# francescovidaich964/TensorNetworkForML

Measured on AMD Instinct MI355X. Metric: sweep-steps/sec, 28x28 MNIST-shaped, bond=20, batch=5000 per GPU, higher is better.
Workload: dtype f32; 1 GPU; c3: N=784 sites, D=2, L=2, bond 20, batch 5000/GPU, softmax+full_cross_ent, trunc=fixed, L2_flag=True; pass = hand-over of one of 4 staged batches + forward + 783-step sweep; global_batch=5000, sweep_steps_per_pass=783, parallelism=dp1, distinct_batches=4

## Files before the change

### tensornetworkforml_amd/csrc/kernels_narrow.hip

```cpp
#include "tnml_internal.h"
#include "jacobi_device.h"
#include "small_gemm_device.h"
#include "wide_pipe_device.h"

namespace tnml {

__device__ inline double wave_sum_f64(double v) {
  v += dpp_f64<0xB1>(v);
  v += dpp_f64<0x4E>(v);
  v += dpp_f64<0x141>(v);
  v += dpp_f64<0x140>(v);
  const double r0 = wave_read_f64(v, 0), r1 = wave_read_f64(v, 16), r2 = wave_read_f64(v, 32), r3 = wave_read_f64(v, 48);
  return (r0 + r1) + (r2 + r3);
}

template <int BUF>
__device__ inline void block_sum3(double &a, double &b, double &c, double *scratch) {
  const int lane = threadIdx.x & 63, wave = threadIdx.x >> 6, nw = blockDim.x >> 6;
  double *s = scratch + BUF * 64;
  a = wave_sum_f64(a); b = wave_sum_f64(b); c = wave_sum_f64(c);
  if (lane == 0) { s[wave] = a; s[16 + wave] = b; s[32 + wave] = c; }
  lds_barrier();
  const int w = lane & 15;
  double ta = w < nw ? s[w] : 0.0, tb = w < nw ? s[16 + w] : 0.0, tc = w < nw ? s[32 + w] : 0.0;
// ... 792 lines not shown
        if (round_idx - __builtin_amdgcn_readfirstlane(last_big1) >= ne - 1) { converged = 1; break; }
      }
      if (!converged) kept2 = kept_scale(Gc);
    }
  } else {
    converged = 1;
  }
  double *V = V0;
  if (vLaneOk) {
#pragma unroll
    for (int r = 0; r < kVR; ++r) {
      const int P = vP0 + r;
      if (r < vr && P < np) {
        *reinterpret_cast<double2 *>(V + (2 * P) * ne + 2 * vQ) = make_double2(vb[r][0], vb[r][1]);
        *reinterpret_cast<double2 *>(V + (2 * P + 1) * ne + 2 * vQ) = make_double2(vb[r][2], vb[r][3]);
      }
    }
  }
  if (p.stamps && tid == 0) t_c2 = __builtin_amdgcn_s_memtime();

  for (int j = tid; j < n; j += NT) k.dLam[j] = __builtin_amdgcn_ldexp(fmax(Gc[j * ne + j], 0.0), sc_exp);
  lds_barrier();
  if (use_chol) {
    for (int j = tid; j < n; j += NT) {
      const double ls = Gc[j * ne + j];
      k.dSq[j] = ls > 1e-300 ? 1.0 / sqrt(ls) : 0.0;
    }
    lds_barrier();
    mm_lds(1, n, n, n, Lm, 0, 1, ne, V, 0, ne, 1, [&](int, int i, int j, double v) { Gn[i * ne + j] = v * k.dSq[j]; });
    V = Gn;
    lds_barrier();
  }
  for (int j = wave_u; j < n; j += NT >> 6) {
    const int i = tid & 63;
    const double lj = k.dLam[j];
    const double li = i < n ? k.dLam[i] : 0.0;
    const int rank = __popcll(__ballot(i < n && ((li > lj) || (li == lj && i < j))));
    if (i == 0) {
      k.sOrd[rank] = j;
      if (p.dbg) p.dbg[4 * (size_t)Bs + rank] = sqrt(lj);
    }
  }
  if (tid == 0) {
    if (p.counters) {
      atomicAdd(p.counters, (unsigned long long)sweeps);
      atomicAdd(p.counters + 1, 1ull);
      atomicAdd(p.counters + 2, (unsigned long long)round_idx);
      if (use_chol) atomicAdd(p.counters + 3, 1ull);
    }
    if (!converged) atomicOr(p.status, 2);
    if (p.dbg) {
      double *sc = p.dbg + 4 * (size_t)Bs + kDbgSigma;
      sc[3] = (double)sweeps;
      sc[4] = (double)n;
    }
  }
  lds_barrier();

  if (p.stamps && tid == 0) t_c2b = __builtin_amdgcn_s_memtime();
  int mk = m, ob_s_h = p.ob_s_h, ob_s_d = p.ob_s_d, oa_s_d = p.oa_s_d, oa_s_g = p.oa_s_g;
  const int ob_s_m = p.ob_s_m, oa_s_m = p.oa_s_m;
  float *const out_behind = p.out_behind, *const out_ahead = p.out_ahead;
  double *const Nh_new = p.Nh_new;
  if (p.trunc_thr > 0.0) {
    if (tid == 0) {
      double tot = 0.0;
      for (int j = 0; j < n; ++j) tot += sqrt(k.dLam[k.sOrd[j]]);
      double cum = 0.0;
      int idx = 0;
      bool found = false;
      for (int j = 0; j < n && !found; ++j) {
        cum += sqrt(k.dLam[k.sOrd[j]]);
// ... 13 lines not shown
    const double lam = k.dLam[k.sOrd[sp]];
    const bool ok = lam > 1e-300 && lam > 1e-30 * lam_max;
    const double sq = ok ? sqrt(sqrt(lam)) : 0.0;
    k.dSq[sp] = sq;
    k.dSq[ne + sp] = ok ? 1.0 / sq : 0.0;
  }
  lds_barrier();
  for (int kk = wave_u; kk < n; kk += NT >> 6)
   for (int sp = tid & 63; sp < mk; sp += 64) {
    const int j = k.sOrd[sp];
    const double vq = V[kk * ne + j];
    const float v = (float)(vq * k.dSq[sp]);
    k.dVs[kk * mk + sp] = vq * k.dSq[ne + sp];
    if (short_rows) {
      k.sCb[kk * mk + sp] = v;
      if (p.persist) PL.Ad[kk * mk + sp] = vq * k.dSq[sp];
      st_behind((kk / D) * ob_s_h + (kk % D) * ob_s_d + sp * ob_s_m, v);
    } else {
      const int l = kk % L, q = kk / L;
      out_ahead[sp * oa_s_m + (q / g) * oa_s_d + (q % g) * oa_s_g + l] = v;
    }
   }
  lds_barrier();
  const int DM = D * mk;
  auto store_T2 = [&](int, int i, int j, double v) { k.dT2[i * DM + j] = v; };
  if (short_rows) {
    int slot = 0;
    if (!p.persist || p.write_ahead)
      slot = mm_lds(L, D * g, mk, n, k.fB, 1, L, c, k.dVs, 0, mk, 1,
           [&](int l, int qq, int sp, double acc) {
             const int dk1 = qq >= g ? 1 : 0;
             out_ahead[__mul24(sp, oa_s_m) + dk1 * oa_s_d + __mul24(qq - dk1 * g, oa_s_g) + l] = (float)acc;
           });
    if (Nh_new) mm_lds(1, h, DM, h, k.dNh, 0, h, 1, k.sCb, 0, DM, 1, store_T2, false, slot);
  } else {
    mm_lds(D, h, mk, n, k.fBp, c + 1, D * (c + 1), 1, k.dVs, 0, mk, 1,
           [&](int dk, int h_, int sp, double acc) {
             const float v = (float)acc;
             k.sCb[__mul24(h_ * D + dk, mk) + sp] = v;
             if (p.persist) PL.Ad[__mul24(h_ * D + dk, mk) + sp] = acc;
             st_behind(__mul24(h_, ob_s_h) + dk * ob_s_d + __mul24(sp, ob_s_m), v);
           });
  }
  lds_barrier();
  if (p.persist) {
    if (wave_u == (NT >> 6) - 1) {
      const int ln = tid & 63;
      const __amdgpu_buffer_rsrc_t rP = sc1_rsrc(p.Apub);
      for (int e = ln; e < (r * mk) >> 1; e += 64) st_sc1_b128(rP, (unsigned)e * 16u, pack_d2(PL.Ad[2 * e], PL.Ad[2 * e + 1]));
      for (int e = ln; e < (mk + 1) >> 1; e += 64) {
        const double i0 = k.dSq[ne + 2 * e], i1 = 2 * e + 1 < mk ? k.dSq[ne + 2 * e + 1] : 0.0;
        st_sc1_b128(rP, (unsigned)(r * mk + 2 * e) * 8u, pack_d2(i0 * i0, i1 * i1));
      }
      asm volatile("s_waitcnt vmcnt(0)" ::: "memory");
      if (ln == 0) { unsigned *const aflag = p.aflag; __hip_atomic_store(aflag, (unsigned)p.coretoken, __ATOMIC_RELAXED, __HIP_MEMORY_SCOPE_AGENT); }
    }
  }

  if (p.stamps && tid == 0) t_c2c = __builtin_amdgcn_s_memtime();
  if (Nh_new) {
    if (!short_rows) {
      mm_lds(1, h, DM, h, k.dNh, 0, h, 1, k.sCb, 0, DM, 1, store_T2);
      lds_barrier();
    }
    mm_lds(1, mk, mk, h * D, k.sCb, 0, 1, mk, k.dT2, 0, mk, 1,
           [&](int, int i, int j, double v) {
             Nh_new[i * mk + j] = v;
             if (p.persist) PL.Nh[i * mk + j] = v;
           });
    if (p.persist) {
      lds_barrier();
      const __amdgpu_buffer_rsrc_t rP = sc1_rsrc(p.Apub);
      const int oN = persist_pub_off(r * mk, mk), nn2 = mk * mk;
      for (int e = tid; e < (nn2 + 1) >> 1; e += NT)
        st_sc1_b128(rP, (unsigned)(oN + 2 * e) * 8u, pack_d2(PL.Nh[2 * e], 2 * e + 1 < nn2 ? PL.Nh[2 * e + 1] : 0.0));
    }
  }

  if (p.stamps && tid == 0) {
    const unsigned long long t_c3 = __builtin_amdgcn_s_memtime(), t_r3 = __builtin_amdgcn_s_memrealtime();
    p.stamps[0] = (double)(t_c1 - t_c0); p.stamps[1] = (double)(t_c2 - t_c1); p.stamps[2] = (double)(t_c3 - t_c2);
    p.stamps[3] = (double)(t_r3 - t_r0); p.stamps[4] = (double)sweeps; p.stamps[5] = (double)n;
    p.stamps[50] = (double)round_idx;
    for (int i = 0; i < 5; ++i) p.stamps[9 + i] = (double)(t_p[i] - (i ? t_p[i - 1] : t_c0));
    p.stamps[6] = (double)(t_c2b - t_c2); p.stamps[7] = (double)(t_c2c - t_c2b); p.stamps[8] = (double)(t_c3 - t_c2c);
  }

  if (tid == 0 && p.metrics) {
    const double cnt = (double)ldtail(3);
    const double inv = cnt > 0 ? 1.0 / cnt : 0.0;
    p.metrics[0] = (float)((double)ldtail(0) * inv);
// ... 117 lines not shown
      const int nT = nr * DG * L;
      double *Tdst = t.T + (size_t)r0 * DG * L, *Ndst = t.TN + (size_t)r0 * DG * L;
      for (int e = tid; e < nT; e += NT) __hip_atomic_store(Tdst + e, oT[e], __ATOMIC_RELAXED, __HIP_MEMORY_SCOPE_AGENT);
      if (t.l2_flag) {
        lds_barrier();
        for (int e = tid; e < nT; e += NT) __hip_atomic_store(Ndst + e, oN[e], __ATOMIC_RELAXED, __HIP_MEMORY_SCOPE_AGENT);
      }
    }
    asm volatile("s_waitcnt vmcnt(0)" ::: "memory");
    lds_barrier();
    if (tid == 0) __hip_atomic_fetch_add(t.tcnt, 1u, __ATOMIC_RELAXED, __HIP_MEMORY_SCOPE_AGENT);
    return false;
  }
  const int cw = (RW + nH - 1) / nH, c0 = min(RW, hid * cw), nc = min(RW, c0 + cw) - c0;
  const int cw2 = 2 * cw;
  double *sA = (double *)smem_raw;
  double *sIv = sA + (((size_t)zr * h + 1) & ~(size_t)1);
  double *sNh = sIv + ((h + 1) & ~1);
  double *sS = sNh + (((size_t)h * h + 1) & ~(size_t)1);
  float *sOut = (float *)(sS + persist_helper_ss_doubles(zr, h, cw));
  double *sP2 = (double *)sOut + (size_t)h * cw;
  float *sZf = (float *)(sP2 + (size_t)h * cw);
  float *sAff = sZf + (size_t)zr * cw;
  double *hst = (t.stamps && hid == 0 && tid == 0) ? t.stamps : nullptr;
  double *hst2 = (t.stamps && hid == 0) ? t.stamps : nullptr;
  auto rt = []() { return (double)(__builtin_amdgcn_s_memrealtime() & ((1ull << 40) - 1)); };
  if (tid == 0) { if (hst) hst[22] = rt(); give_up(spin_wait_ge(t.tcnt, (unsigned)nH, t.abort_flag)); if (hst) hst[30] = rt(); }
  lds_barrier();
  if (sBad) return true;
  for (int e = tid; e < zr * nc; e += NT) {
    const int i = e / nc, cc = e - i * nc;
    const size_t src = (size_t)i * RW + c0 + cc;
    sS[i * cw2 + cc] = __hip_atomic_load(t.T + src, __ATOMIC_RELAXED, __HIP_MEMORY_SCOPE_AGENT);
    sS[i * cw2 + cw + cc] = t.l2_flag ? __hip_atomic_load(t.TN + src, __ATOMIC_RELAXED, __HIP_MEMORY_SCOPE_AGENT) : 0.0;
  }
  lds_barrier();
  if (tid == 0) { give_up(spin_wait_ge(t.zready, t.zwant, t.abort_flag)); if (hst) hst[24] = rt(); }
  lds_barrier();
  if (sBad) return true;
  for (int e = tid; e < zr * nc; e += NT) {
    const int i = e / nc, cc = e - i * nc;
    sZf[i * cw + cc] = ld_sc1(t.Z + (size_t)i * RW + c0 + cc);
  }
  lds_barrier();
  if (tid == 0) { give_up(t.awant ? spin_wait_ge(t.aflag, t.awant, t.abort_flag) : 0); if (hst) hst[23] = rt(); }
  lds_barrier();
  if (sBad) return true;
  if (t.awant) {
    const __amdgpu_buffer_rsrc_t rP = sc1_rsrc(t.Apub);
    const int n1 = persist_pub_off(zr * h, h) >> 1, nA = (zr * h) >> 1;
    for (int e = tid; e < n1; e += NT) {
      const tn_uvec4 q = ld_sc1_b128(rP, (unsigned)e * 16u);
      *reinterpret_cast<tn_uvec4 *>(sA + 2 * e) = q;
      if (e < nA) { const dvec2_t a = __builtin_bit_cast(dvec2_t, q); sAff[2 * e] = (float)a[0]; sAff[2 * e + 1] = (float)a[1]; }
    }
  } else if (tid == 0) {
    sA[0] = 1.0; sAff[0] = 1.f; sIv[0] = 1.0; sNh[0] = 1.0;
  }
  lds_barrier();
  if (hst) hst[25] = rt();
  if (nc > 0) {
    mm_lds_f32(h, nc, zr, sAff, 1, h, sZf, cw, 1, [&](int i, int j, float v) { sOut[i * cw + j] = v; });
    const int slot = (((h + 15) >> 4) * ((nc + 15) >> 4)) & ((NT >> 6) - 1);
    mm_lds(1, h, t.l2_flag ? 2 * cw : cw, zr, sA, 0, 1, h, sS, 0, cw2, 1,
           [&](int, int i, int j, double v) {
             if (j < cw) { if (j < nc) sOut[(h + i) * cw + j] = (float)(v * sIv[i]); }
             else sP2[i * cw + (j - cw)] = v * sIv[i];
           }, false, slot);
  }
  if (t.l2_flag) {
    if (t.awant && (tid >> 6) == (NT >> 6) - 1) {
      const int ln = tid & 63;
      int bad = 0;
      if (ln == 0) { if (hst2) hst2[31] = rt(); bad = spin_wait_ge(t.nflag, t.awant, t.abort_flag); give_up(bad); if (hst2) hst2[21] = rt(); }
      if (!__builtin_amdgcn_readfirstlane(bad)) {
        const __amdgpu_buffer_rsrc_t rP = sc1_rsrc(t.Apub);
        const int oN = persist_pub_off(zr * h, h), nq = (h * h + 1) >> 1;
        for (int e0 = ln; e0 < nq; e0 += 4 * 64) {
          tn_uvec4 q[4];
#pragma unroll
          for (int u = 0; u < 4; ++u) if (e0 + 64 * u < nq) q[u] = ld_sc1_b128(rP, (unsigned)(oN + 2 * (e0 + 64 * u)) * 8u);
#pragma unroll
          for (int u = 0; u < 4; ++u) if (e0 + 64 * u < nq) *reinterpret_cast<tn_uvec4 *>(sNh + 2 * (e0 + 64 * u)) = q[u];
        }
      }
    }
  }
  lds_barrier();
  if (t.l2_flag && sBad) return true;
  st_sc1_rows(t.prepRaw, sOut, h, cw, RW, c0, nc);
  st_sc1_rows(t.prepB, sOut + (size_t)h * cw, h, cw, RW, c0, nc);
  if (t.l2_flag) {
    if (nc > 0) {
      mm_lds(1, h, nc, h, sNh, 0, 1, h, sP2, 0, cw, 1, [&](int, int i, int j, double v) { sS[i * cw + j] = v; });
    }
    lds_barrier();
    st_sc1_rows(t.prepG, sS, h, cw, RW, c0, nc);
  }
  if (hst) hst[26] = rt();
  asm volatile("s_waitcnt vmcnt(0)" ::: "memory");
  lds_barrier();
  if (tid == 0) __hip_atomic_fetch_add(t.pcnt, 1u, __ATOMIC_RELAXED, __HIP_MEMORY_SCOPE_AGENT);
  if (hst) hst[27] = rt();
  return false;
}

__global__ __launch_bounds__(kNarrowThreads) void sweep_persist_kernel(const PersistStep *__restrict__ steps_g, int n_steps, int nH) {
// ... 109 lines not shown
```

### tensornetworkforml_amd/csrc/san/hip_stub.cpp

```cpp
#include <hip/hip_runtime.h>
#include <rccl/rccl.h>
#include <sys/mman.h>
#include <cstdarg>
#include <cstdio>
#include <cstdlib>
#include <cstring>
#include <map>
#include <string>
#include <vector>
#include <cxxabi.h>
#include "../tnml_internal.h"
#include "../wide_pipe_device.h"

using namespace tnml;

namespace san {
static char *g_base = nullptr;
static size_t g_used = 0;
static constexpr size_t kArena = (size_t)1 << 38, kGap = (size_t)1 << 20;
static std::map<uintptr_t, size_t> &alloc_map() { static auto *m = new std::map<uintptr_t, size_t>; return *m; }
static std::map<const void *, std::string> &kernel_map() { static auto *m = new std::map<const void *, std::string>; return *m; }
static std::map<std::string, long> &launch_map() { static auto *m = new std::map<std::string, long>; return *m; }
#define g_alloc alloc_map()
#define g_kernels kernel_map()
// ... 87 lines not shown
  if (p.m_out) { need(p.m_out, 4, "NarrowParams.m_out"); memcpy(p.m_out, &p.m, 4); }
  opt(p.metrics, 2 * 4, "NarrowParams.metrics"); opt(p.counters, 4 * 8, "NarrowParams.counters") ; need(p.status, 4, "NarrowParams.status");
  if (p.pipe) {
    need(p.zred, (size_t)(p.zsize + kMetricSlots) * 4, "NarrowParams.zred");
    if (!p.z_first && !p.persist) need(p.zcore.base, view_extent(p.zcore, 1) * 4, "NarrowParams.zcore");
    opt(p.flag, 4, "NarrowParams.flag");
  }
  if (p.fused) {
    opt(p.slabs, (size_t)p.nslabs * p.slab_stride * 4, "NarrowParams.slabs");
    opt(p.prepB, (size_t)p.bsize * 4, "NarrowParams.prepB"); opt(p.prepG, (size_t)p.bsize * 8, "NarrowParams.prepG");
    need(p.sync, 4, "NarrowParams.sync");
  }
  if (p.persist) {
    need(p.prepB, (size_t)p.bsize * 4, "NarrowParams.prepB (persistent)"); need(p.prepG, (size_t)p.bsize * 8, "NarrowParams.prepG (persistent)");
    need(p.pready, 4, "NarrowParams.pready"); need(p.aflag, 4, "NarrowParams.aflag"); need(p.coreflag, 4, "NarrowParams.coreflag"); need(p.abort_flag, 4, "NarrowParams.abort_flag");
    need(p.Apub, persist_pub_doubles(kD * p.h * p.m, p.m) * 8, "NarrowParams.Apub");
  }
}
static void check_pipe(const WidePipeParams &w) {
  scan(&w, sizeof w, "WidePipeParams");
  const size_t bp = w.b_pad;
  if (w.b < 1 || w.b > w.b_pad || w.b_pad % 64 || w.ntiles != w.b_pad / kTS) die("WidePipeParams: b %d b_pad %d ntiles %d", w.b, w.b_pad, w.ntiles);
  if (!w.first) {
    need(w.x_j, bp * kD * 4, "WidePipeParams.x_j");
    if (w.do_ext) {
      need(w.Ecur, (size_t)w.hj * bp * 4, "WidePipeParams.Ecur (written)");
      need(w.x_jm1, bp * kD * 4, "WidePipeParams.x_jm1");
      if (!w.first_ext) need(w.Eprev, (size_t)w.hprev * bp * 4, "WidePipeParams.Eprev");
      need(w.ext_core.base, view_extent(w.ext_core, 1) * 4, "WidePipeParams.ext_core");
    } else opt(w.Ecur, (size_t)w.hj * bp * 4, "WidePipeParams.Ecur (read)");
    if (w.do_f) { opt(w.Gj, (size_t)w.gj * bp * 4, "WidePipeParams.Gj"); need(w.Bnew, (size_t)w.hj * kD * kD * w.gj * w.L * 4, "WidePipeParams.Bnew"); }
// ... 75 lines not shown
  P(prepG) P(sync) R(trunc_thr) I(left_dir) P(m_out) R(chol_thr) R(svd_stop2) P(status) I(wait_count) I(pipe) I(z_first) I(z_rows)
  I(zsize) P(zred) V(zcore) P(flag) I(token) I(persist) I(write_ahead) I(persist_off) I(Mcap) P(prepRaw) P(pready) I(pwant) P(Apub)
  P(aflag) P(coreflag) I(coretoken) P(zpoll_flag) I(zpoll_want) P(done_flag) I(done_val) P(abort_flag)
}
static void tr_struct(const WideParams &p) {
  I(b) I(b_pad) I(L) I(h) I(g) I(hp) I(gp) I(do_f) I(do_ext) I(first_ext) I(act_fn) I(loss_fn) R(T) P(x_km1) P(x_k) P(x_kp1) P(Hprev)
  P(Hcur) P(Gprev) P(Gcur) P(Bprev) V(ext_core) P(y) P(f) P(slabs) I(slab_stride) I(bsize) P(stamps)
}
static void tr_struct(const WidePipeParams &p) {
  I(b) I(b_pad) I(L) I(hj) I(gj) I(gn) I(hprev) I(first) I(do_ext) I(first_ext) I(do_f) I(wait_flag) I(do_z) I(act_fn) I(loss_fn) R(T)
  P(x_jm1) P(x_j) P(x_jp1) P(x_jp2) P(Eprev) P(Ecur) V(ext_core) P(Gj) P(Gn) P(Bnew) P(y) P(f) I(zsize) I(slab_stride) P(slabs) P(gslabs)
  P(zred) P(gcnt) P(tcnt) I(nwide) I(gsz) I(ngroups) I(one_level) I(wg0) I(tiles_per_wg) I(ntiles) P(flag) I(token) P(status) I(persist)
  P(coreflag) I(corewant) P(zready) I(zpublish) P(abort_flag) P(stamps)
}
static void tr_struct(const PersistHelperParams &p) {
  I(zr) I(s) I(g) I(L) I(h) I(l2_flag) P(W) V(lab) V(pl) P(Ng) P(T) P(TN) P(Z) P(prepRaw) P(prepB) P(prepG) P(Apub) P(flag) I(want)
  P(aflag) P(nflag) I(awant) P(zready) I(zwant) P(tcnt) P(pcnt) P(abort_flag) P(status) P(stamps)
}
static void tr_struct(const PersistStep &p) { tr(" n:"); tr_struct(p.n); tr(" w:"); tr_struct(p.w); tr(" t:"); tr_struct(p.t); }
static void tr_struct(const PrepParams &p) { V(lab) V(pl) P(Nh) P(Ng) I(h) I(g) I(s) I(L) I(l2_flag) P(prepB) P(prepG) I(nparts) }
static void tr_struct(const MeetParams &p) { P(Lenv) P(Renv) P(x) P(core) P(f) I(b) I(b_pad) I(ml) I(mr) I(D) I(L) I(rows_per_chunk) }
static void tr_struct(const BigExtArgs &p) { P(Eprev) P(x_km1) P(x_k) V(A) I(b_pad) P(Ecur) P(Pk) }
static void tr_struct(const ChainSite &p) { I(core_off) I(is_label) I(n_in) I(n_out) I(s_in) I(s_d) I(s_out) I(x_site) I(env_out_off) }
static void tr_struct(const NormChainSite &p) { I(core_off) I(n_in) I(n_out) I(s_in) I(s_d) I(s_out) I(env_out_off) }
#undef I
#undef R
#undef P
#undef V
template <class S> static void tr_rows(const char *what, const S *rows, int n) {
  for (int i = 0; i < n; ++i) { tr("  %s %d:", what, i); tr_struct(rows[i]); tr("\n"); }
}
static void tr_launch(const std::string &name, dim3 g, dim3 b, size_t shm, hipStream_t st, void **args) {
// ... 284 lines not shown
```

### tensornetworkforml_amd/csrc/tnml_api.hip

```cpp
#include <rccl/rccl.h>

#include <algorithm>
#include <cmath>
#include <cstdarg>
#include <cstdio>
#include <cstring>
#include <cstdlib>

#include "tnml_internal.h"
#include "small_gemm_device.h"
#include "wide_pipe_device.h"

using namespace tnml;

static thread_local std::string g_err;

static int fail(int code, const char *fmt, ...) {
  char buf[1024];
  va_list ap;
  va_start(ap, fmt);
  vsnprintf(buf, sizeof buf, fmt, ap);
  va_end(ap);
  g_err = buf;
  return code;
// ... 274 lines not shown
  HIP_TRY(hipMalloc(&c->prepB, c->bmax * sizeof(float)));
  HIP_TRY(hipMalloc(&c->prepG, c->bmax * sizeof(double)));
  HIP_TRY(hipMalloc(&c->sync, sizeof(unsigned)));
  HIP_TRY(hipMemset(c->sync, 0, sizeof(unsigned)));
  c->zstride = (int)((2 * c->bmax + kMetricSlots + 63) / 64 * 64);
  HIP_TRY(hipMalloc(&c->gslabs, (size_t)kPipeGroupMax * c->zstride * sizeof(float)));
  HIP_TRY(hipMalloc(&c->zred, (size_t)c->zstride * sizeof(float)));
  HIP_TRY(hipMalloc(&c->pipe.cnt, 32 * sizeof(unsigned)));
  HIP_TRY(hipMemset(c->pipe.cnt, 0, 32 * sizeof(unsigned)));
  HIP_TRY(hipMalloc(&c->zred2, (size_t)c->zstride * sizeof(float)));
  HIP_TRY(hipMalloc(&c->Tbuf[0], (size_t)c->zstride * sizeof(double)));
  HIP_TRY(hipMalloc(&c->Tbuf[1], (size_t)c->zstride * sizeof(double)));
  HIP_TRY(hipMalloc(&c->TNbuf[0], (size_t)c->zstride * sizeof(double)));
  HIP_TRY(hipMalloc(&c->TNbuf[1], (size_t)c->zstride * sizeof(double)));
  HIP_TRY(hipMalloc(&c->prepRaw, c->bmax * sizeof(float)));
  HIP_TRY(hipMalloc(&c->Apub, persist_pub_doubles(D * Mmax * Mmax, Mmax) * sizeof(double)));
  HIP_TRY(hipMalloc(&c->pst_dev, (size_t)(N + 1) * sizeof(PersistStep)));
  for (int i = 0; i < 2; ++i) {
    HIP_TRY(hipHostMalloc(&c->pst_host[i], (size_t)(N + 1) * sizeof(PersistStep)));
    HIP_TRY(hipEventCreateWithFlags(&c->pst_ev[i], hipEventDisableTiming));
  }
  HIP_TRY(hipMalloc(&c->pst_cnt, (size_t)(N + 1) * 32 * sizeof(unsigned)));
  HIP_TRY(hipMalloc(&c->pst_flags, 8 * sizeof(unsigned)));
  HIP_TRY(hipMalloc(&c->Bscr2, c->bmax * sizeof(float)));
  HIP_TRY(hipMalloc(&c->red, (size_t)c->slab_stride * sizeof(float)));
  c->metrics_cap = N;
  HIP_TRY(hipMalloc(&c->metrics, (size_t)c->metrics_cap * 2 * sizeof(float)));
  HIP_TRY(hipMalloc(&c->scal, 64 * sizeof(float)));
  c->dbg_elems = 4 * c->bmax + kDbgSigma + kDbgScalars + 8;
  HIP_TRY(hipMalloc(&c->dbg, c->dbg_elems * sizeof(double)));
  HIP_TRY(hipMalloc(&c->status, 2 * sizeof(int)));
// ... 1253 lines not shown
  if (1 + nH + nwide > c->num_cus) return 0;
  const int Mcap = c->Mmax;
  const size_t pbytes = persist_lds_bytes(Mcap);
  unsigned *fl = c->pst_flags;
  float *zr2[2] = {c->zred, c->zred2};
  size_t lds_narrow = 0, lds_wide = 0, lds_help = 0;
  fill_wide_pipe(c, pro, sc, -1);
  pro.do_ext = 0; pro.wait_flag = 0; pro.do_z = 1; pro.do_f = 0;
  set_pipe_tiles(pro, tpw);
  pro.wg0 = 1 + nH; pro.persist = 1; pro.zred = zr2[0]; pro.zready = fl + 2; pro.zpublish = 1; pro.abort_flag = fl + 4;
  pro.gcnt = c->pst_cnt + (size_t)n_steps * 32; pro.tcnt = pro.gcnt + 16;
  if (!wide_pipe_fits(c, pro)) return give_up();
  pipe_try_one_level(pro);
  lds_wide = wide_pipe_lds_bytes(pro);
  double bytes = 0, flops = 0;
  for (int k = 0; k < n_steps; ++k) {
    const StepGeom q = step_geom(c, left_dir, trunc_policy);
    if (q.fail) return give_up();
    const int h = q.h, g = q.g, s = q.s, m = q.m;
    const size_t nlds = narrow_lds_bytes(h, g, s, L, m);
    if (q.nn > 64 || (q.nn & 1) || nlds + pbytes > kLdsMax || h > Mcap || m > Mcap || q.bsize > 8192) return give_up();
    PersistStep &ps = st[k];
    ps = PersistStep{};
    NarrowParams &n = ps.n;
    fill_update(c, n, q, sc.l2_flag, sc.lr, sc.weight_dec);
    n.out_ahead = c->lab[(c->lab_cur + (n_steps - k)) & 1];
    n.write_ahead = (k == n_steps - 1);
    n.metrics = c->metrics + 2 * (size_t)k;
    n.chol_thr = c->chol_thr;
    n.stamps = (c->stamps && k == n_steps / 2) ? c->dbg + 4 * c->bmax + kDbgSigma + 5 : nullptr;
// ... 17 lines not shown
    set_pipe_tiles(wp, tpw);
    wp.wg0 = 1 + nH; wp.persist = 1; wp.flag = fl + 0; wp.token = (unsigned)k + 1;
    wp.coreflag = fl + 3; wp.corewant = (unsigned)k; wp.zready = fl + 2; wp.zpublish = (unsigned)k + 2; wp.abort_flag = fl + 4;
    wp.zred = zr2[(k + 1) & 1];
    wp.gcnt = c->pst_cnt + (size_t)k * 32; wp.tcnt = wp.gcnt + 16;
    wp.stamps = n.stamps;
    if (!wide_pipe_fits(c, wp)) return give_up();
    pipe_try_one_level(wp);
    lds_wide = std::max(lds_wide, wide_pipe_lds_bytes(wp));
    PersistHelperParams &t = ps.t;
    t.zr = zr; t.s = s; t.g = g; t.L = L; t.h = h; t.l2_flag = n.l2_flag;
    t.W = k == 0 ? nullptr : c->Bnew;
    t.lab = n.lab; t.pl = n.pl; t.Ng = n.Ng;
    t.T = c->Tbuf[k & 1]; t.TN = c->TNbuf[k & 1]; t.Z = zr2[k & 1];
    t.prepRaw = c->prepRaw; t.prepB = c->prepB; t.prepG = c->prepG; t.Apub = c->Apub;
    t.flag = fl + 0; t.want = (unsigned)k; t.aflag = fl + 5; t.nflag = fl + 3; t.awant = (unsigned)k; t.zready = fl + 2; t.zwant = (unsigned)k + 1;
    t.tcnt = c->pst_cnt + (size_t)k * 32 + 20; t.pcnt = c->pst_cnt + (size_t)k * 32 + 21;
    t.abort_flag = fl + 4; t.status = c->status; t.stamps = n.stamps;
    lds_help = std::max(lds_help, persist_helper_lds_bytes(zr, s, g, L, h, nH));
    if ((size_t)zr * D * D * g * L + kMetricSlots > (size_t)c->zstride) return give_up();
    advance_frame(c, q, m);
    if (!c->stamps || k <= n_steps / 2) note_last_step(c, q);
    add_step_work(c, q, bytes, flops);
  }
  const size_t lds = c->persist_mode >= 2 ? lds_narrow + pbytes : std::max(std::max(lds_narrow + pbytes, lds_wide), lds_help);
  if (lds > kLdsMax || lds_wide > kLdsMax || lds_help > kLdsMax) return give_up();
  const int persist_off = (int)((lds - pbytes) & ~(size_t)15);
  for (int k = 0; k < n_steps; ++k) st[k].n.persist_off = persist_off;
  HIP_TRY(hipMemcpyAsync(c->pst_dev, st, (size_t)(n_steps + 1) * sizeof(PersistStep), hipMemcpyHostToDevice, c->stream));
  HIP_TRY(hipEventRecord(c->pst_ev[buf], c->stream));
  c->pst_cur ^= 1;
  HIP_TRY(hipMemsetAsync(c->pst_flags, 0, 8 * sizeof(unsigned), c->stream));
  HIP_TRY(hipMemsetAsync(c->pst_cnt, 0, (size_t)(n_steps + 1) * 32 * sizeof(unsigned), c->stream));
  if (c->persist_mode >= 2) {
    HIP_TRY(hipEventRecord(c->ev_p0, c->stream));
    HIP_TRY(hipStreamWaitEvent(c->stream2, c->ev_p0, 0));
    HIP_TRY(hipStreamWaitEvent(c->stream3, c->ev_p0, 0));
    launch_sweep_persist_split(c->pst_dev, n_steps, nH, nwide, lds, lds_help, lds_wide, c->stream, c->stream2, c->stream3);
    HIP_TRY(hipGetLastError());
    HIP_TRY(hipEventRecord(c->ev_p2, c->stream2));
    HIP_TRY(hipEventRecord(c->ev_p3, c->stream3));
    HIP_TRY(hipStreamWaitEvent(c->stream, c->ev_p2, 0));
    HIP_TRY(hipStreamWaitEvent(c->stream, c->ev_p3, 0));
// ... 816 lines not shown
```

### tensornetworkforml_amd/csrc/tnml_internal.h

```cpp
#pragma once
#include <hip/hip_runtime.h>
#include <stdint.h>

#include <string>
#include <vector>

#include "../../include/tnml.h"

namespace tnml {

constexpr int kD = 2;
constexpr int kMaxD = 8;
constexpr int kTS = 32;
constexpr int kWideThreads = 1024;
constexpr int kNarrowThreads = 1024;
constexpr int kMetricSlots = 4;
constexpr int kDbgScalars = 120 + 16 * 12;
constexpr int kDbgSigma = 128;
constexpr double kCholThrSmall = 0.35;
constexpr double kCholThrDefault = 0.22;
constexpr double kSvdStop2Default = 1e-6;
constexpr int kCounterSlots = 16;

struct CoreView {
// ... 86 lines not shown
  int write_ahead;
  int persist_off;
  int Mcap;
  const float *prepRaw;
  const unsigned *pready;
  unsigned pwant;
  double *Apub;
  unsigned *aflag;
  unsigned *coreflag;
  unsigned coretoken;
  const unsigned *zpoll_flag; unsigned zpoll_want;
  unsigned *done_flag; unsigned done_val;
  unsigned *abort_flag;
};

struct PersistLds { double *Nh, *Ad; };
__host__ __device__ inline PersistLds persist_lds(unsigned char *base, int Mcap) {
  PersistLds q;
  q.Nh = (double *)base;
  q.Ad = q.Nh + (size_t)Mcap * Mcap;
  return q;
}
inline size_t persist_lds_bytes(int Mcap) {
  return ((size_t)Mcap * Mcap + (size_t)kD * Mcap * Mcap) * sizeof(double) + 16;
}

struct NormChainSite {
  int core_off;
  int n_in, n_out, s_in, s_d, s_out;
  long long env_out_off;
};

void launch_transpose_input(const float *X_bnd, float *X_nbd, int b, int b_pad, int N, hipStream_t st);
void launch_env_chain(const ChainSite *sites_dev, int n_sites, const float *cores, const float *labcore,
                      const float *X, float *env_base, float *f, int b, int b_pad, int L, int Mmax,
                      float *logmax_out, hipStream_t st, bool force_plain = false);
constexpr int kChainSamplesPerBlock = 16;
struct MeetParams {
  const float *Lenv, *Renv;
// ... 92 lines not shown
```

### tensornetworkforml_amd/csrc/wide_pipe_device.h

```cpp
#pragma once
#include "tnml_internal.h"
#include "act_device.h"
#include "jacobi_device.h"

namespace tnml {

typedef float fvec4 __attribute__((ext_vector_type(4)));
constexpr int kPipeThreads = 1024;
constexpr int kPTSP = kTS + 1;
constexpr int kPipeGroupMax = 16;

__host__ __device__ inline int upm(int x, int m) { return (x + m - 1) / m * m; }

__device__ inline void st_sc1(float *p, float v) { __hip_atomic_store(p, v, __ATOMIC_RELAXED, __HIP_MEMORY_SCOPE_AGENT); }
__device__ inline float ld_sc1(const float *p) { return __hip_atomic_load(p, __ATOMIC_RELAXED, __HIP_MEMORY_SCOPE_AGENT); }

struct WidePipeParams {
  int b, b_pad, L;
  int hj, gj;
  int gn;
  int hprev;
  int first;
  int do_ext;
  int first_ext;
// ... 104 lines not shown
}
void launch_step_pipe(const NarrowParams &p, const WidePipeParams &w, size_t lds_bytes, hipStream_t st);
void launch_step_pipe_update(const NarrowParams &p, const WidePipeParams &w, size_t lds_bytes, hipStream_t st);

struct PersistHelperParams {
  int zr, s, g, L, h;
  int l2_flag;
  const float *W;
  CoreView lab, pl;
  const double *Ng;
  double *T, *TN;
  const float *Z;
  float *prepRaw, *prepB;
  double *prepG;
  const double *Apub;
  const unsigned *flag;
  unsigned want;
  const unsigned *aflag;
  const unsigned *nflag;
  unsigned awant;
  const unsigned *zready;
  unsigned zwant;
  unsigned *tcnt, *pcnt;
  unsigned *abort_flag;
  int *status;
  double *stamps;
};
struct PersistStep { NarrowParams n; WidePipeParams w; PersistHelperParams t; };
constexpr int kPersistHelpers = 8;
__host__ __device__ inline int persist_pub_off(int na, int h) { return ((na + 1) & ~1) + ((h + 1) & ~1); }
__host__ __device__ inline size_t persist_pub_doubles(int na, int h) { return (size_t)persist_pub_off(na, h) + (((size_t)h * h + 1) & ~(size_t)1); }
__host__ __device__ inline size_t persist_helper_ss_doubles(int zr, int h, int cw) {
  const size_t a = 2 * (size_t)zr * cw, b = (size_t)h * cw;
  return ((a > b ? a : b) + 1) & ~(size_t)1;
}
inline size_t persist_helper_lds_bytes(int zr, int s, int g, int L, int h, int nH) {
  const size_t DG = (size_t)kD * g, RW = kD * DG * L;
  const size_t per = ((size_t)zr * kD + nH - 1) / nH, cw = (RW + nH - 1) / nH;
  const size_t p1 = (((per * s * L + 3) & ~(size_t)3) + (((size_t)s * DG + 3) & ~(size_t)3)) * sizeof(float) +
                    ((((size_t)g * g + 1) & ~(size_t)1) + 2 * per * DG * L) * sizeof(double);
  const size_t p2 = (persist_pub_doubles(zr * h, h) + persist_helper_ss_doubles(zr, h, (int)cw) + 2 * (size_t)h * cw) * sizeof(double) +
                    ((size_t)zr * cw + (size_t)zr * h) * sizeof(float);
  return (p1 > p2 ? p1 : p2) + 64;
}
void launch_sweep_persist(const PersistStep *steps_dev, int n_steps, int n_helpers, int grid, size_t lds_bytes, hipStream_t st);
void launch_sweep_persist_split(const PersistStep *steps_dev, int n_steps, int n_helpers, int n_wide, size_t lds_update, size_t lds_helper,
                                size_t lds_wide, hipStream_t st_update, hipStream_t st_helper, hipStream_t st_wide);


template <int PERSIST>
struct WidePipeArgs : WidePipeParams {
  __device__ __forceinline__ WidePipeArgs(const WidePipeParams &q) : WidePipeParams(q) {}
  static constexpr int persist = PERSIST;
};
template <class WP>
__device__ __forceinline__ bool wide_pipe_block(const WP &p, float *smem) {
  const WidePipeDims dm = wide_pipe_dims(p);
  const WidePipeSmem w = wide_pipe_carve(smem, p, dm);
// ... 360 lines not shown
```

Baseline: 21160 sweep-steps/s.

## Publish raw eigenvectors early so persistent helpers rebuild A and Nh themselves

The narrow update block now publishes the Jacobi eigenvector matrix and eigenvalues to the shared buffer right after diagonalisation and raises the ready flag then, instead of after computing the scaled A and the new Nh. Helper blocks read V and lambda, sort and scale them, and for long rows multiply by the previous core themselves. They also compute the Nh recurrence locally, which removes the separate nflag wait. This lets helpers start earlier and overlap with the narrow block's remaining work, at the cost of duplicated sorting and GEMM work in every helper and more LDS.

```diff
diff --git a/tensornetworkforml_amd/csrc/kernels_narrow.hip b/tensornetworkforml_amd/csrc/kernels_narrow.hip
--- a/tensornetworkforml_amd/csrc/kernels_narrow.hip
+++ b/tensornetworkforml_amd/csrc/kernels_narrow.hip
@@ -830,13 +830,32 @@
       if (r < vr && P < np) {
         *reinterpret_cast<double2 *>(V + (2 * P) * ne + 2 * vQ) = make_double2(vb[r][0], vb[r][1]);
         *reinterpret_cast<double2 *>(V + (2 * P + 1) * ne + 2 * vQ) = make_double2(vb[r][2], vb[r][3]);
+        if (p.persist && !use_chol) {
+          const __amdgpu_buffer_rsrc_t rP = sc1_rsrc((double *)p.Apub);
+          st_sc1_b128(rP, (unsigned)((2 * P) * ne + 2 * vQ) * 8u, pack_d2(vb[r][0], vb[r][1]));
+          st_sc1_b128(rP, (unsigned)((2 * P + 1) * ne + 2 * vQ) * 8u, pack_d2(vb[r][2], vb[r][3]));
+        }
       }
     }
   }
   if (p.stamps && tid == 0) t_c2 = __builtin_amdgcn_s_memtime();
 
   for (int j = tid; j < n; j += NT) k.dLam[j] = __builtin_amdgcn_ldexp(fmax(Gc[j * ne + j], 0.0), sc_exp);
-  lds_barrier();
+  auto publish_lam = [&]() {
+    const __amdgpu_buffer_rsrc_t rP = sc1_rsrc((double *)p.Apub);
+    for (int e = tid; e < ne >> 1; e += NT) {
+      const int j0 = 2 * e, j1 = 2 * e + 1;
+      const double l0 = __builtin_amdgcn_ldexp(fmax(Gc[j0 * ne + j0], 0.0), sc_exp);
+      const double l1 = j1 < n ? __builtin_amdgcn_ldexp(fmax(Gc[j1 * ne + j1], 0.0), sc_exp) : 0.0;
+      st_sc1_b128(rP, (unsigned)(persist_pub_off(ne) + j0) * 8u, pack_d2(l0, l1));
+    }
+  };
+  if (p.persist && !use_chol) {
+    publish_lam();
+    asm volatile("s_waitcnt vmcnt(0)" ::: "memory");
+  }
+  lds_barrier();
+  if (p.persist && !use_chol && tid == 0) { unsigned *const aflag = p.aflag; __hip_atomic_store(aflag, (unsigned)p.coretoken, __ATOMIC_RELAXED, __HIP_MEMORY_SCOPE_AGENT); }
   if (use_chol) {
     for (int j = tid; j < n; j += NT) {
       const double ls = Gc[j * ne + j];
@@ -846,6 +865,12 @@
     mm_lds(1, n, n, n, Lm, 0, 1, ne, V, 0, ne, 1, [&](int, int i, int j, double v) { Gn[i * ne + j] = v * k.dSq[j]; });
     V = Gn;
     lds_barrier();
+    if (p.persist) {
+      const __amdgpu_buffer_rsrc_t rP = sc1_rsrc((double *)p.Apub);
+      for (int e = tid; e < (ne * ne) >> 1; e += NT) st_sc1_b128(rP, (unsigned)e * 16u, pack_d2(V[2 * e], V[2 * e + 1]));
+      publish_lam();
+      asm volatile("s_waitcnt vmcnt(0)" ::: "memory");
+    }
   }
   for (int j = wave_u; j < n; j += NT >> 6) {
     const int i = tid & 63;
@@ -872,6 +897,7 @@
     }
   }
   lds_barrier();
+  if (p.persist && use_chol && tid == 0) { unsigned *const aflag = p.aflag; __hip_atomic_store(aflag, (unsigned)p.coretoken, __ATOMIC_RELAXED, __HIP_MEMORY_SCOPE_AGENT); }
 
   if (p.stamps && tid == 0) t_c2b = __builtin_amdgcn_s_memtime();
   int mk = m, ob_s_h = p.ob_s_h, ob_s_d = p.ob_s_d, oa_s_d = p.oa_s_d, oa_s_g = p.oa_s_g;
@@ -915,7 +941,6 @@
     k.dVs[kk * mk + sp] = vq * k.dSq[ne + sp];
     if (short_rows) {
       k.sCb[kk * mk + sp] = v;
-      if (p.persist) PL.Ad[kk * mk + sp] = vq * k.dSq[sp];
       st_behind((kk / D) * ob_s_h + (kk % D) * ob_s_d + sp * ob_s_m, v);
     } else {
       const int l = kk % L, q = kk / L;
@@ -939,25 +964,10 @@
            [&](int dk, int h_, int sp, double acc) {
              const float v = (float)acc;
              k.sCb[__mul24(h_ * D + dk, mk) + sp] = v;
-             if (p.persist) PL.Ad[__mul24(h_ * D + dk, mk) + sp] = acc;
              st_behind(__mul24(h_, ob_s_h) + dk * ob_s_d + __mul24(sp, ob_s_m), v);
            });
   }
   lds_barrier();
-  if (p.persist) {
-    if (wave_u == (NT >> 6) - 1) {
-      const int ln = tid & 63;
-      const __amdgpu_buffer_rsrc_t rP = sc1_rsrc(p.Apub);
-      for (int e = ln; e < (r * mk) >> 1; e += 64) st_sc1_b128(rP, (unsigned)e * 16u, pack_d2(PL.Ad[2 * e], PL.Ad[2 * e + 1]));
-      for (int e = ln; e < (mk + 1) >> 1; e += 64) {
-        const double i0 = k.dSq[ne + 2 * e], i1 = 2 * e + 1 < mk ? k.dSq[ne + 2 * e + 1] : 0.0;
-        st_sc1_b128(rP, (unsigned)(r * mk + 2 * e) * 8u, pack_d2(i0 * i0, i1 * i1));
-      }
-      asm volatile("s_waitcnt vmcnt(0)" ::: "memory");
-      if (ln == 0) { unsigned *const aflag = p.aflag; __hip_atomic_store(aflag, (unsigned)p.coretoken, __ATOMIC_RELAXED, __HIP_MEMORY_SCOPE_AGENT); }
-    }
-  }
-
   if (p.stamps && tid == 0) t_c2c = __builtin_amdgcn_s_memtime();
   if (Nh_new) {
     if (!short_rows) {
@@ -969,13 +979,6 @@
              Nh_new[i * mk + j] = v;
              if (p.persist) PL.Nh[i * mk + j] = v;
            });
-    if (p.persist) {
-      lds_barrier();
-      const __amdgpu_buffer_rsrc_t rP = sc1_rsrc(p.Apub);
-      const int oN = persist_pub_off(r * mk, mk), nn2 = mk * mk;
-      for (int e = tid; e < (nn2 + 1) >> 1; e += NT)
-        st_sc1_b128(rP, (unsigned)(oN + 2 * e) * 8u, pack_d2(PL.Nh[2 * e], 2 * e + 1 < nn2 ? PL.Nh[2 * e + 1] : 0.0));
-    }
   }
 
   if (p.stamps && tid == 0) {
@@ -1123,16 +1126,19 @@
   }
   const int cw = (RW + nH - 1) / nH, c0 = min(RW, hid * cw), nc = min(RW, c0 + cw) - c0;
   const int cw2 = 2 * cw;
+  const int wave_u = __builtin_amdgcn_readfirstlane(tid >> 6);
+  const int pn = t.pn, pc = t.pc, hp = zr / D;
+  const bool long_rows = zr > pc;
   double *sA = (double *)smem_raw;
   double *sIv = sA + (((size_t)zr * h + 1) & ~(size_t)1);
-  double *sNh = sIv + ((h + 1) & ~1);
-  double *sS = sNh + (((size_t)h * h + 1) & ~(size_t)1);
+  double *sS = sIv + ((h + 1) & ~1);
   float *sOut = (float *)(sS + persist_helper_ss_doubles(zr, h, cw));
   double *sP2 = (double *)sOut + (size_t)h * cw;
   float *sZf = (float *)(sP2 + (size_t)h * cw);
   float *sAff = sZf + (size_t)zr * cw;
+  const PersistHelperCore hc = persist_helper_core((unsigned char *)(sZf + ((((size_t)zr * cw + (size_t)zr * h) + 3) & ~(size_t)3)), zr, h, pn, pc);
+  double *sNh = (double *)(smem_raw + t.nh_off);
   double *hst = (t.stamps && hid == 0 && tid == 0) ? t.stamps : nullptr;
-  double *hst2 = (t.stamps && hid == 0) ? t.stamps : nullptr;
   auto rt = []() { return (double)(__builtin_amdgcn_s_memrealtime() & ((1ull << 40) - 1)); };
   if (tid == 0) { if (hst) hst[22] = rt(); give_up(spin_wait_ge(t.tcnt, (unsigned)nH, t.abort_flag)); if (hst) hst[30] = rt(); }
   lds_barrier();
@@ -1143,6 +1149,12 @@
     sS[i * cw2 + cc] = __hip_atomic_load(t.T + src, __ATOMIC_RELAXED, __HIP_MEMORY_SCOPE_AGENT);
     sS[i * cw2 + cw + cc] = t.l2_flag ? __hip_atomic_load(t.TN + src, __ATOMIC_RELAXED, __HIP_MEMORY_SCOPE_AGENT) : 0.0;
   }
+  if (t.awant && long_rows) {
+    for (int e = tid; e < zr * pc; e += NT) {
+      const int i = e / pc, x = e - i * pc;
+      hc.sBp[i * (pc + 1) + x] = ld_sc1(t.W + e);
+    }
+  }
   lds_barrier();
   if (tid == 0) { give_up(spin_wait_ge(t.zready, t.zwant, t.abort_flag)); if (hst) hst[24] = rt(); }
   lds_barrier();
@@ -1157,49 +1169,87 @@
   if (sBad) return true;
   if (t.awant) {
     const __amdgpu_buffer_rsrc_t rP = sc1_rsrc(t.Apub);
-    const int n1 = persist_pub_off(zr * h, h) >> 1, nA = (zr * h) >> 1;
-    for (int e = tid; e < n1; e += NT) {
-      const tn_uvec4 q = ld_sc1_b128(rP, (unsigned)e * 16u);
-      *reinterpret_cast<tn_uvec4 *>(sA + 2 * e) = q;
-      if (e < nA) { const dvec2_t a = __builtin_bit_cast(dvec2_t, q); sAff[2 * e] = (float)a[0]; sAff[2 * e + 1] = (float)a[1]; }
-    }
-  } else if (tid == 0) {
-    sA[0] = 1.0; sAff[0] = 1.f; sIv[0] = 1.0; sNh[0] = 1.0;
+    const int n1 = (int)(persist_pub_doubles(pn) >> 1);
+    for (int e0 = tid; e0 < n1; e0 += 2 * NT) {
+      tn_uvec4 q[2];
+#pragma unroll
+      for (int u = 0; u < 2; ++u) if (e0 + u * NT < n1) q[u] = ld_sc1_b128(rP, (unsigned)(e0 + u * NT) * 16u);
+#pragma unroll
+      for (int u = 0; u < 2; ++u) if (e0 + u * NT < n1) *reinterpret_cast<tn_uvec4 *>(hc.sV + 2 * (e0 + u * NT)) = q[u];
+    }
+    lds_barrier();
+    for (int j = wave_u; j < pn; j += NT >> 6) {
+      const int i = tid & 63;
+      const double lj = hc.sLam[j];
+      const double li = i < pn ? hc.sLam[i] : 0.0;
+      const int rank = __popcll(__ballot(i < pn && ((li > lj) || (li == lj && i < j))));
+      if (i == 0) hc.sOrd[rank] = j;
+    }
+    lds_barrier();
+    const double lam_max = hc.sLam[hc.sOrd[0]];
+    auto col_scale = [&](int sp, double &sq, double &isq) {
+      const double lam = hc.sLam[hc.sOrd[sp]];
+      const bool ok = lam > 1e-300 && lam > 1e-30 * lam_max;
+      sq = ok ? sqrt(sqrt(lam)) : 0.0;
+      isq = ok ? 1.0 / sq : 0.0;
+    };
+    if (!long_rows) {
+      for (int kk = wave_u; kk < pn; kk += NT >> 6)
+        for (int sp = tid & 63; sp < h; sp += 64) {
+          double sq, isq;
+          col_scale(sp, sq, isq);
+          const double vq = hc.sV[kk * pn + hc.sOrd[sp]];
+          const double a = vq * sq;
+          sA[kk * h + sp] = a;
+          sAff[kk * h + sp] = (float)a;
+          if (kk == 0) sIv[sp] = isq * isq;
+        }
+    } else {
+      for (int kk = wave_u; kk < pn; kk += NT >> 6)
+        for (int sp = tid & 63; sp < h; sp += 64) {
+          double sq, isq;
+          col_scale(sp, sq, isq);
+          hc.sVs[kk * h + sp] = hc.sV[kk * pn + hc.sOrd[sp]] * isq;
+          if (kk == 0) sIv[sp] = isq * isq;
+        }
+      lds_barrier();
+      mm_lds(D, hp, h, pn, hc.sBp, pc + 1, D * (pc + 1), 1, hc.sVs, 0, h, 1,
+             [&](int dk, int h_, int sp, double acc) {
+               sA[__mul24(h_ * D + dk, h) + sp] = acc;
+               sAff[__mul24(h_ * D + dk, h) + sp] = (float)acc;
+             });
+    }
+  } else {
+    if (tid == 0) { sA[0] = 1.0; sAff[0] = 1.f; sIv[0] = 1.0; }
+    if (t.l2_flag) for (int e = tid; e < h * h; e += NT) sNh[e] = t.Nh ? t.Nh[e] : 1.0;
   }
   lds_barrier();
   if (hst) hst[25] = rt();
-  if (nc > 0) {
-    mm_lds_f32(h, nc, zr, sAff, 1, h, sZf, cw, 1, [&](int i, int j, float v) { sOut[i * cw + j] = v; });
-    const int slot = (((h + 15) >> 4) * ((nc + 15) >> 4)) & ((NT >> 6) - 1);
-    mm_lds(1, h, t.l2_flag ? 2 * cw : cw, zr, sA, 0, 1, h, sS, 0, cw2, 1,
-           [&](int, int i, int j, double v) {
-             if (j < cw) { if (j < nc) sOut[(h + i) * cw + j] = (float)(v * sIv[i]); }
-             else sP2[i * cw + (j - cw)] = v * sIv[i];
-           }, false, slot);
-  }
-  if (t.l2_flag) {
-    if (t.awant && (tid >> 6) == (NT >> 6) - 1) {
-      const int ln = tid & 63;
-      int bad = 0;
-      if (ln == 0) { if (hst2) hst2[31] = rt(); bad = spin_wait_ge(t.nflag, t.awant, t.abort_flag); give_up(bad); if (hst2) hst2[21] = rt(); }
-      if (!__builtin_amdgcn_readfirstlane(bad)) {
-        const __amdgpu_buffer_rsrc_t rP = sc1_rsrc(t.Apub);
-        const int oN = persist_pub_off(zr * h, h), nq = (h * h + 1) >> 1;
-        for (int e0 = ln; e0 < nq; e0 += 4 * 64) {
-          tn_uvec4 q[4];
-#pragma unroll
-          for (int u = 0; u < 4; ++u) if (e0 + 64 * u < nq) q[u] = ld_sc1_b128(rP, (unsigned)(oN + 2 * (e0 + 64 * u)) * 8u);
-#pragma unroll
-          for (int u = 0; u < 4; ++u) if (e0 + 64 * u < nq) *reinterpret_cast<tn_uvec4 *>(sNh + 2 * (e0 + 64 * u)) = q[u];
-        }
-      }
-    }
-  }
-  lds_barrier();
-  if (t.l2_flag && sBad) return true;
+  const int DM = D * h;
+  {
+    int slot = 0;
+    if (nc > 0) {
+      mm_lds_f32(h, nc, zr, sAff, 1, h, sZf, cw, 1, [&](int i, int j, float v) { sOut[i * cw + j] = v; });
+      slot = (((h + 15) >> 4) * ((nc + 15) >> 4)) & ((NT >> 6) - 1);
+      slot = mm_lds(1, h, t.l2_flag ? 2 * cw : cw, zr, sA, 0, 1, h, sS, 0, cw2, 1,
+                    [&](int, int i, int j, double v) {
+                      if (j < cw) { if (j < nc) sOut[(h + i) * cw + j] = (float)(v * sIv[i]); }
+                      else sP2[i * cw + (j - cw)] = v * sIv[i];
+                    }, false, slot);
+    }
+    if (t.l2_flag && t.awant)
+      mm_lds(1, hp, DM, hp, sNh, 0, hp, 1, sAff, 0, DM, 1, [&](int, int i, int j, double v) { hc.sT2[i * DM + j] = v; }, false, slot);
+  }
+  lds_barrier();
+  if (hst) hst[31] = rt();
   st_sc1_rows(t.prepRaw, sOut, h, cw, RW, c0, nc);
   st_sc1_rows(t.prepB, sOut + (size_t)h * cw, h, cw, RW, c0, nc);
   if (t.l2_flag) {
+    if (t.awant) {
+      mm_lds(1, h, h, zr, sAff, 0, 1, h, hc.sT2, 0, h, 1, [&](int, int i, int j, double v) { sNh[i * h + j] = v; });
+      lds_barrier();
+    }
+    if (hst) hst[21] = rt();
     if (nc > 0) {
       mm_lds(1, h, nc, h, sNh, 0, 1, h, sP2, 0, cw, 1, [&](int, int i, int j, double v) { sS[i * cw + j] = v; });
     }
diff --git a/tensornetworkforml_amd/csrc/san/hip_stub.cpp b/tensornetworkforml_amd/csrc/san/hip_stub.cpp
--- a/tensornetworkforml_amd/csrc/san/hip_stub.cpp
+++ b/tensornetworkforml_amd/csrc/san/hip_stub.cpp
@@ -125,7 +125,7 @@
   if (p.persist) {
     need(p.prepB, (size_t)p.bsize * 4, "NarrowParams.prepB (persistent)"); need(p.prepG, (size_t)p.bsize * 8, "NarrowParams.prepG (persistent)");
     need(p.pready, 4, "NarrowParams.pready"); need(p.aflag, 4, "NarrowParams.aflag"); need(p.coreflag, 4, "NarrowParams.coreflag"); need(p.abort_flag, 4, "NarrowParams.abort_flag");
-    need(p.Apub, persist_pub_doubles(kD * p.h * p.m, p.m) * 8, "NarrowParams.Apub");
+    { const int r = kD * p.h, cc = kD * p.g * p.L, n = r <= cc ? r : cc; need(p.Apub, persist_pub_doubles(n + (n & 1)) * 8, "NarrowParams.Apub"); }
   }
 }
 static void check_pipe(const WidePipeParams &w) {
@@ -231,8 +231,8 @@
   P(coreflag) I(corewant) P(zready) I(zpublish) P(abort_flag) P(stamps)
 }
 static void tr_struct(const PersistHelperParams &p) {
-  I(zr) I(s) I(g) I(L) I(h) I(l2_flag) P(W) V(lab) V(pl) P(Ng) P(T) P(TN) P(Z) P(prepRaw) P(prepB) P(prepG) P(Apub) P(flag) I(want)
-  P(aflag) P(nflag) I(awant) P(zready) I(zwant) P(tcnt) P(pcnt) P(abort_flag) P(status) P(stamps)
+  I(zr) I(s) I(g) I(L) I(h) I(l2_flag) P(W) V(lab) V(pl) P(Ng) P(T) P(TN) P(Z) P(prepRaw) P(prepB) P(prepG) P(Apub) I(pn) I(pc) P(Nh) I(nh_off) P(flag) I(want)
+  P(aflag) I(awant) P(zready) I(zwant) P(tcnt) P(pcnt) P(abort_flag) P(status) P(stamps)
 }
 static void tr_struct(const PersistStep &p) { tr(" n:"); tr_struct(p.n); tr(" w:"); tr_struct(p.w); tr(" t:"); tr_struct(p.t); }
 static void tr_struct(const PrepParams &p) { V(lab) V(pl) P(Nh) P(Ng) I(h) I(g) I(s) I(L) I(l2_flag) P(prepB) P(prepG) I(nparts) }
diff --git a/tensornetworkforml_amd/csrc/tnml_api.hip b/tensornetworkforml_amd/csrc/tnml_api.hip
--- a/tensornetworkforml_amd/csrc/tnml_api.hip
+++ b/tensornetworkforml_amd/csrc/tnml_api.hip
@@ -312,7 +312,7 @@
   HIP_TRY(hipMalloc(&c->TNbuf[0], (size_t)c->zstride * sizeof(double)));
   HIP_TRY(hipMalloc(&c->TNbuf[1], (size_t)c->zstride * sizeof(double)));
   HIP_TRY(hipMalloc(&c->prepRaw, c->bmax * sizeof(float)));
-  HIP_TRY(hipMalloc(&c->Apub, persist_pub_doubles(D * Mmax * Mmax, Mmax) * sizeof(double)));
+  HIP_TRY(hipMalloc(&c->Apub, persist_pub_doubles(64) * sizeof(double)));
   HIP_TRY(hipMalloc(&c->pst_dev, (size_t)(N + 1) * sizeof(PersistStep)));
   for (int i = 0; i < 2; ++i) {
     HIP_TRY(hipHostMalloc(&c->pst_host[i], (size_t)(N + 1) * sizeof(PersistStep)));
@@ -1596,6 +1596,7 @@
   pipe_try_one_level(pro);
   lds_wide = wide_pipe_lds_bytes(pro);
   double bytes = 0, flops = 0;
+  int prev_nn = 0, prev_cols = 0;
   for (int k = 0; k < n_steps; ++k) {
     const StepGeom q = step_geom(c, left_dir, trunc_policy);
     if (q.fail) return give_up();
@@ -1643,19 +1644,23 @@
     t.lab = n.lab; t.pl = n.pl; t.Ng = n.Ng;
     t.T = c->Tbuf[k & 1]; t.TN = c->TNbuf[k & 1]; t.Z = zr2[k & 1];
     t.prepRaw = c->prepRaw; t.prepB = c->prepB; t.prepG = c->prepG; t.Apub = c->Apub;
-    t.flag = fl + 0; t.want = (unsigned)k; t.aflag = fl + 5; t.nflag = fl + 3; t.awant = (unsigned)k; t.zready = fl + 2; t.zwant = (unsigned)k + 1;
+    t.flag = fl + 0; t.want = (unsigned)k; t.aflag = fl + 5; t.awant = (unsigned)k; t.zready = fl + 2; t.zwant = (unsigned)k + 1;
     t.tcnt = c->pst_cnt + (size_t)k * 32 + 20; t.pcnt = c->pst_cnt + (size_t)k * 32 + 21;
     t.abort_flag = fl + 4; t.status = c->status; t.stamps = n.stamps;
-    lds_help = std::max(lds_help, persist_helper_lds_bytes(zr, s, g, L, h, nH));
+    t.pn = prev_nn; t.pc = prev_cols; t.Nh = k == 0 ? n.Nh : nullptr;
+    lds_help = std::max(lds_help, persist_helper_lds_bytes(zr, s, g, L, h, nH, prev_nn, prev_cols));
+    prev_nn = q.nn; prev_cols = D * g * L;
     if ((size_t)zr * D * D * g * L + kMetricSlots > (size_t)c->zstride) return give_up();
     advance_frame(c, q, m);
     if (!c->stamps || k <= n_steps / 2) note_last_step(c, q);
     add_step_work(c, q, bytes, flops);
   }
+  const int nh_off = (int)lds_help;
+  lds_help += (size_t)Mcap * Mcap * sizeof(double);
   const size_t lds = c->persist_mode >= 2 ? lds_narrow + pbytes : std::max(std::max(lds_narrow + pbytes, lds_wide), lds_help);
   if (lds > kLdsMax || lds_wide > kLdsMax || lds_help > kLdsMax) return give_up();
   const int persist_off = (int)((lds - pbytes) & ~(size_t)15);
-  for (int k = 0; k < n_steps; ++k) st[k].n.persist_off = persist_off;
+  for (int k = 0; k < n_steps; ++k) { st[k].n.persist_off = persist_off; st[k].t.nh_off = nh_off; }
   HIP_TRY(hipMemcpyAsync(c->pst_dev, st, (size_t)(n_steps + 1) * sizeof(PersistStep), hipMemcpyHostToDevice, c->stream));
   HIP_TRY(hipEventRecord(c->pst_ev[buf], c->stream));
   c->pst_cur ^= 1;
diff --git a/tensornetworkforml_amd/csrc/tnml_internal.h b/tensornetworkforml_amd/csrc/tnml_internal.h
--- a/tensornetworkforml_amd/csrc/tnml_internal.h
+++ b/tensornetworkforml_amd/csrc/tnml_internal.h
@@ -124,15 +124,14 @@
   unsigned *abort_flag;
 };
 
-struct PersistLds { double *Nh, *Ad; };
+struct PersistLds { double *Nh; };
 __host__ __device__ inline PersistLds persist_lds(unsigned char *base, int Mcap) {
   PersistLds q;
   q.Nh = (double *)base;
-  q.Ad = q.Nh + (size_t)Mcap * Mcap;
   return q;
 }
 inline size_t persist_lds_bytes(int Mcap) {
-  return ((size_t)Mcap * Mcap + (size_t)kD * Mcap * Mcap) * sizeof(double) + 16;
+  return (size_t)Mcap * Mcap * sizeof(double) + 16;
 }
 
 struct NormChainSite {
diff --git a/tensornetworkforml_amd/csrc/wide_pipe_device.h b/tensornetworkforml_amd/csrc/wide_pipe_device.h
--- a/tensornetworkforml_amd/csrc/wide_pipe_device.h
+++ b/tensornetworkforml_amd/csrc/wide_pipe_device.h
@@ -142,10 +142,12 @@
   float *prepRaw, *prepB;
   double *prepG;
   const double *Apub;
+  int pn, pc;
+  const double *Nh;
+  int nh_off;
   const unsigned *flag;
   unsigned want;
   const unsigned *aflag;
-  const unsigned *nflag;
   unsigned awant;
   const unsigned *zready;
   unsigned zwant;
@@ -156,20 +158,37 @@
 };
 struct PersistStep { NarrowParams n; WidePipeParams w; PersistHelperParams t; };
 constexpr int kPersistHelpers = 8;
-__host__ __device__ inline int persist_pub_off(int na, int h) { return ((na + 1) & ~1) + ((h + 1) & ~1); }
-__host__ __device__ inline size_t persist_pub_doubles(int na, int h) { return (size_t)persist_pub_off(na, h) + (((size_t)h * h + 1) & ~(size_t)1); }
+__host__ __device__ inline int persist_pub_off(int ne) { return ne * ne; }
+__host__ __device__ inline size_t persist_pub_doubles(int ne) { return (size_t)ne * ne + (size_t)ne; }
 __host__ __device__ inline size_t persist_helper_ss_doubles(int zr, int h, int cw) {
   const size_t a = 2 * (size_t)zr * cw, b = (size_t)h * cw;
   return ((a > b ? a : b) + 1) & ~(size_t)1;
 }
-inline size_t persist_helper_lds_bytes(int zr, int s, int g, int L, int h, int nH) {
+struct PersistHelperCore { double *sV, *sLam, *sSq, *sT2, *sVs; float *sBp; int *sOrd; size_t bytes; };
+__host__ __device__ inline PersistHelperCore persist_helper_core(unsigned char *base, int zr, int h, int pn, int pc) {
+  PersistHelperCore q;
+  const bool long_rows = zr > pc;
+  double *d = (double *)base;
+  q.sV = d; d += (size_t)pn * pn;
+  q.sLam = d; d += pn;
+  q.sSq = d; d += 2 * (size_t)((h + 1) & ~1);
+  q.sT2 = d; d += ((size_t)zr * h + 1) & ~(size_t)1;
+  q.sVs = d; d += long_rows ? (((size_t)pn * h + 1) & ~(size_t)1) : 0;
+  float *f = (float *)d;
+  q.sBp = f; f += long_rows ? (((size_t)zr * (pc + 1) + 3) & ~(size_t)3) : 0;
+  q.sOrd = (int *)f;
+  q.bytes = (size_t)((unsigned char *)(q.sOrd + ((pn + 3) & ~3)) - base);
+  return q;
+}
+inline size_t persist_helper_lds_bytes(int zr, int s, int g, int L, int h, int nH, int pn, int pc) {
   const size_t DG = (size_t)kD * g, RW = kD * DG * L;
   const size_t per = ((size_t)zr * kD + nH - 1) / nH, cw = (RW + nH - 1) / nH;
   const size_t p1 = (((per * s * L + 3) & ~(size_t)3) + (((size_t)s * DG + 3) & ~(size_t)3)) * sizeof(float) +
                     ((((size_t)g * g + 1) & ~(size_t)1) + 2 * per * DG * L) * sizeof(double);
-  const size_t p2 = (persist_pub_doubles(zr * h, h) + persist_helper_ss_doubles(zr, h, (int)cw) + 2 * (size_t)h * cw) * sizeof(double) +
-                    ((size_t)zr * cw + (size_t)zr * h) * sizeof(float);
-  return (p1 > p2 ? p1 : p2) + 64;
+  alignas(16) static unsigned char origin[16];
+  const size_t p2 = ((((size_t)zr * h + 1) & ~(size_t)1) + ((h + 1) & ~1) + persist_helper_ss_doubles(zr, h, (int)cw) + 2 * (size_t)h * cw) * sizeof(double) +
+                    ((((size_t)zr * cw + (size_t)zr * h) + 3) & ~(size_t)3) * sizeof(float) + persist_helper_core(origin, zr, h, pn, pc).bytes;
+  return (((p1 > p2 ? p1 : p2) + 15) & ~(size_t)15) + 64;
 }
 void launch_sweep_persist(const PersistStep *steps_dev, int n_steps, int n_helpers, int grid, size_t lds_bytes, hipStream_t st);
 void launch_sweep_persist_split(const PersistStep *steps_dev, int n_steps, int n_helpers, int n_wide, size_t lds_update, size_t lds_helper,
```

New measurement: 20860 sweep-steps/s. -1.4%, worse.
